# aliyun/heif-decoder-lib

Measured on AMD Instinct MI355X. Metric: megapixels/sec HEIC grid->RGB24, higher is better.
Workload: dtype u8

## Files before the change

heif-decoder-lib_amd/csrc/batch.cpp:

```cpp
#include <cstdio>
#include <algorithm>
#include <cmath>
#include <cstdlib>
#include <cstring>
#include <map>
#include <memory>
#include <tuple>
#include <vector>

#include "hm_device.h"
#include "hm_internal.h"
#include "hm_overlap_plan.h"

namespace {

struct DeviceBuffer {
  void* p = nullptr;
  size_t cap = 0;
  int ensure(size_t n)
  {
    if (n <= cap) return HM_OK;
    if (p) hm_pool_device_free(p);
    p = hm_pool_device_alloc(n);
    cap = p ? n : 0;
// ... 700 lines not shown
{
  if (!b) return hm_fail(HM_ERR_INVALID_ARG, "null batch");
  b->colour = false;
  b->tail_state = 0;
  b->col_y.clear(); b->col_cb.clear(); b->col_cr.clear(); b->col_out.clear();
  if (n_images == 0) return HM_OK;
  if (!d || n_images < 0 || !d_y || !d_cb || !d_cr || !d_out) return hm_fail(HM_ERR_INVALID_ARG, "null argument");
  if (b->items.empty() || b->items.size() % (size_t)n_images) return hm_fail(HM_ERR_INVALID_ARG, "%zu pictures do not divide into %d images", b->items.size(), n_images);
  const int pipe = hm_colour_pipeline(d);
  if (pipe < 0) return pipe;
  b->colour_desc = *d;
  b->col_y.assign(d_y, d_y + n_images); b->col_cb.assign(d_cb, d_cb + n_images); b->col_cr.assign(d_cr, d_cr + n_images);
  b->col_out.assign(d_out, d_out + n_images);
  b->colour_chunk = images_per_group;
  b->colour = true;
  return HM_OK;
}

int hm_batch_set_concurrency(hm_batch* b, int groups)
{
  if (!b || groups < 0 || groups > 8) return hm_fail(HM_ERR_INVALID_ARG, "bad argument");
  b->drain();
  b->groups = groups;
  return HM_OK;
}

int hm_batch_last_groups(const hm_batch* b, int* first_cut)
{
  if (!b) return -1;
  if (first_cut) *first_cut = b->last_cut;
  return b->last_groups;
}

int hm_batch_tail_kind(const hm_batch* b) { return b && b->tail_state == 2 ? b->tail_kind : -1; }

int hm_batch_tail_fused(const hm_batch* b) { return b && b->tail_state == 2 ? 1 : 0; }

int hm_batch_set_profiling(hm_batch* b, int slots)
{
  if (!b || slots < 0 || slots > 4096) return hm_fail(HM_ERR_INVALID_ARG, "bad argument");
  b->profiling = slots;
  b->exec_count = 0;
  return HM_OK;
}

static int batch_timings(hm_batch* b, int slot, float ms[5])
{
  if (!b || !ms) return hm_fail(HM_ERR_INVALID_ARG, "null argument");
  ms[0] = ms[1] = ms[2] = ms[3] = ms[4] = 0.f;
  if (!b->profiling || slot < 0 || slot >= b->profiling || slot >= b->exec_count || slot >= (int)b->timelines.size() || b->timelines[slot].used == 0)
    return hm_fail(HM_ERR_INVALID_ARG, "profiling not enabled or slot not recorded");
  const hm_batch::Timeline& t = b->timelines[slot];
  hipError_t e = hipEventSynchronize(t.ev[t.used - 1]);
  if (e != hipSuccess) return hm_check_hip(e, "hipEventSynchronize");
  if (t.spans) {
    std::vector<std::pair<float, float>> iv[5];
    for (size_t i = 1; i < t.used; i++) {
      if (t.kind[i] < 0) continue;
      float t0 = 0.f, t1 = 0.f;
      if ((e = hipEventElapsedTime(&t0, t.ev[0], t.ev[i - 1])) != hipSuccess || (e = hipEventElapsedTime(&t1, t.ev[0], t.ev[i])) != hipSuccess)
        return hm_check_hip(e, "hipEventElapsedTime");
      iv[t.kind[i]].emplace_back(t0, std::max(t0, t1));
    }
    for (int q = 0; q < 5; q++) {
      std::sort(iv[q].begin(), iv[q].end());
      float end = 0.f;
// ... 99 lines not shown
```

heif-decoder-lib_amd/csrc/chain.hip:

```cpp
#include "recon_common.h"

#include <stdlib.h>
#include <atomic>
#include <map>
#include <memory>
#include <mutex>
#include <new>
#include <utility>

#include "hm_internal.h"

namespace {

#ifdef HM_CHAIN_TIMING
#define HM_T_DECL unsigned long long t_prev = __builtin_amdgcn_s_memtime(); unsigned int t_acc[6] = {0, 0, 0, 0, 0, 0}, t_part[4] = {0, 0, 0, 0}; int t_in_svc = 0; (void)t_part; (void)t_in_svc
#if HM_CHAIN_TIMING == 2
#define HM_T_LAP(i) (void)t_prev
#define HM_T_COUNT(i) t_acc[i] += 64
#else
#define HM_T_LAP(i) do { if (HM_CHAIN_TIMING != 4) { const unsigned long long t_now = __builtin_amdgcn_s_memtime(); t_acc[i] += (unsigned int)(t_now - t_prev); t_prev = t_now; } } while (0)
#define HM_T_COUNT(i)
#endif
#if HM_CHAIN_TIMING == 4
#define HM_T_SVC_BEGIN() do { t_prev = __builtin_amdgcn_s_memtime(); t_in_svc = 1; } while (0)
// ... 584 lines not shown
          running = running && (uint32_t)my_off < my_kb;
          left = my_kb == 0 ? 0 : left;
          if (ballot(running) == 0) { __builtin_amdgcn_s_sleep(1); continue; }
        }
      }
    }
    const unsigned long long m_running = ballot(running);
    const int16_t* const my_res = rres + rslot * 16;
    const unsigned long long m_q4 = m_running & ballot((op.y & ((3u << OP_L2_SHIFT) | OP_INTERIOR)) == OP_INTERIOR);
    unsigned long long m_quad = m_q4, s_big = m_running & ~m_q4;
    int n_exec = 1, n_sub = 1;
    bool quad = running && (op.y & ((3u << OP_L2_SHIFT) | OP_INTERIOR)) == OP_INTERIOR;
    if (multi) {
      const uint32_t gq = (uint32_t)((m_q4 & 1) | ((m_q4 >> 15) & 2) | ((m_q4 >> 30) & 4) | ((m_q4 >> 45) & 8));
      const uint32_t gr = (uint32_t)((m_running & 1) | ((m_running >> 15) & 2) | ((m_running >> 30) & 4) | ((m_running >> 45) & 8));
      constexpr bool two = NCL == 1;
      constexpr int SUBX = CAN_LATE ? 2 : SUB;
      auto of_chain = [&](uint32_t m, int c) { return CAN_LATE ? ((m >> (2 * c)) & 3u) : (two ? (((m >> c) & 1u) | (((m >> (c + 2)) & 1u) << 1)) : (c ? 0u : m)); };
      uint32_t run[2], big[2];
#pragma unroll
      for (int c = 0; c < 2; c++) {
        const uint32_t q = of_chain(gq, c), r = of_chain(gr, c);
        run[c] = (uint32_t)__builtin_ctz(~q | (1u << SUBX));
        big[c] = (uint32_t)__builtin_ctz(~((r & ~q) >> run[c]));
      }
      const uint32_t my_run = g == 0 ? run[0] : run[1], my_big = g == 0 ? big[0] : big[1];
      quad = (uint32_t)my_off < my_run;
      m_quad = ballot(quad);
      s_big = ballot((uint32_t)my_off >= my_run && (uint32_t)my_off < my_run + my_big);
      n_exec = (int)(my_run + my_big);
      n_sub = (int)(run[0] > run[1] ? run[0] : run[1]);
    }
    (void)m_quad;
    const unsigned long long s_bres = s_big & ballot((op.y & (OP_CBF | (3u << OP_L2_SHIFT))) == (OP_CBF | (1u << OP_L2_SHIFT)));

    HM_T_LAP(1);
#if defined(HM_Q_PROBE) && (HM_Q_PROBE & 2048)
    if (s_bres && n_pics < 0) {
#else
    if (s_bres) {
#endif
      auto big_res = [&](int gg) -> uint32_t {
        uint32_t idx = (uint32_t)__builtin_amdgcn_readlane((int)op.z, gg * 16) + (uint32_t)lane;
        idx = idx < res_last ? idx : res_last;
        return (uint32_t)(int)resid[idx];
      };
      uint32_t sb_lo = (uint32_t)s_bres, sb_hi = (uint32_t)(s_bres >> 32);
      asm volatile("" : "+s"(sb_lo), "+s"(sb_hi));
      if (sb_lo & 0xFFFFu) bres0 = big_res(0);
      if (sb_lo >> 16) bres1 = big_res(1);
      if (sb_hi & 0xFFFFu) bres2 = big_res(2);
      if (sb_hi >> 16) bres3 = big_res(3);
    }

    HM_MARK("C_begin");
#if defined(HM_Q_PROBE) && (HM_Q_PROBE & 1)
    if (false) {
#else
    if (quad) {
#endif
      if (lane == (int)__builtin_ctzll(ballot(true))) HM_T_COUNT(3);
      const int res_q = (int)my_res[gl];
      const int mode = (int)(op.y & OP_MODE_MASK);
      const int P = Pk;
      Pix* const lp = gbase + (op.x & 0xFFFF);
      const Pix* const tbase = reinterpret_cast<const Pix*>(lds + ((op.y & OP_LINE) ? tl_off : gb_off));
      const Pix* const tc = tbase + (op.x >> 16);
// ... 45 lines not shown
        for (int t = 0; t < n_sub; t++) {
          if (my_off == t) execute();
          WAVE_SYNC();
        }
      }
      else execute();
    }
    WAVE_SYNC();

    HM_T_LAP(2);
    HM_MARK("D_begin");
#if defined(HM_Q_PROBE) && (HM_Q_PROBE & 2)
    for (unsigned long long todo = 0; todo;) {
#else
    for (unsigned long long todo = s_big; todo;) {
#endif
      const int bg = rfl((int)(__builtin_ctzll(todo) >> 4));
      todo &= ~(0xFFFFull << (bg * 16));
      HM_T_COUNT(4);
      const int src = bg * 16;
      const uint32_t ox = (uint32_t)__builtin_amdgcn_readlane((int)op.x, src), oy = (uint32_t)__builtin_amdgcn_readlane((int)op.y, src);
      const uint32_t oz = (uint32_t)__builtin_amdgcn_readlane((int)op.z, src), ow = (uint32_t)__builtin_amdgcn_readlane((int)op.w, src);
      const uint32_t s_gb = (uint32_t)__builtin_amdgcn_readlane((int)gb_off, src), s_tl = (uint32_t)__builtin_amdgcn_readlane((int)tl_off, src);
      const int mode = (int)(oy & OP_MODE_MASK), c = (int)((oy >> OP_C_SHIFT) & 3), log2 = 2 + (int)((oy >> OP_L2_SHIFT) & 3);
      const int path = (int)((oy >> OP_PATH_SHIFT) & 7);
#ifdef HM_D_SKIP
      if ((HM_D_SKIP >> (path != PATH_GEN ? path : 4 + log2)) & 1) continue;
#endif
#if defined(HM_Q_PROBE) && (HM_Q_PROBE & 512)
      const bool cbf = false;
#else
      const bool cbf = (oy & OP_CBF) != 0;
#endif
      const int P = c == 0 ? P0 : P1;
      Pix* const gb = reinterpret_cast<Pix*>(lds + s_gb);
      Pix* const lp = gb + (ox & 0xFFFF);
      const Pix* const tp = reinterpret_cast<const Pix*>(lds + ((oy & OP_LINE) ? s_tl : s_gb)) + (ox >> 16) + 1;
      Pix* const dst = lp + 1;
      const GLOBAL_AS int16_t* const gres = resid + oz;
      const int maxv = (1 << bd) - 1;

      HM_MARK("D_setup_end");
      auto block = [&](auto l2c, auto which) {
        constexpr int L2 = decltype(l2c)::value, WHICH = decltype(which)::value;
        int ln = lane;
        asm volatile("" : "+v"(ln));
        int res_s = 0, res_t[4] = {0, 0, 0, 0};
        const bool pairs = sizeof(Pix) == 1 && L2 >= 4 && WHICH != PATH_B4 && mode >= 2 && mode != 10 && mode != 26;
#ifdef HM_PAIRS_PRE
        uint32_t res_p[2] = {0, 0};
        if (cbf && pairs && L2 == 4) {
#pragma unroll
          for (int t = 0; t < 2; t++) res_p[t] = pairs8_residual<4>(mode >= 18, ln, t, gres);
        }
        else
#endif
        if (cbf && !pairs) {
          if (L2 == 2) {
            const int s_ri = __builtin_amdgcn_readlane((int)ri_me, src);
            const int s_chain = PAIRS ? bg & ((1 << NCL) - 1) : ((CAN_LATE && late) ? bg & 2 : bg);
            res_s = (int)(rres_all + s_chain * (RING * 16) + (s_ri & (RING - 1)) * 16)[ln & 15];
          }
          else if (L2 == 3) {
            uint32_t b = bg == 0 ? bres0 : (bg == 1 ? bres1 : (bg == 2 ? bres2 : bres3));
            asm volatile("" : "+v"(b));
            res_s = (int)b;
          }
          else if (L2 == 4) {
#pragma unroll
            for (int t = 0; t < 4; t++) res_t[t] = (int)gres[ln + 64 * t];
          }
        }
        auto emit = [&](int p, int x, int y, int v) {
          if (cbf) {
            int r;
            if (L2 <= 3) r = res_s;
            else if (L2 == 4) {
              const int t = rfl(p >> 6);
              r = t == 0 ? res_t[0] : (t == 1 ? res_t[1] : (t == 2 ? res_t[2] : res_t[3]));
            }
            else r = (int)gres[p];
            v = clip3i(0, maxv, v + r);
          }
          dst[mul24(y, P) + x] = (Pix)v;
        };
        Blk<Pix> B;
        B.mode = mode; B.c = c; B.bd = bd; B.log2 = L2; B.tskip = 0; B.qp = 0; B.n_coeff = 0; B.P = P;
        const bool smoothed = L2 != 2 && c == 0 && ((filter_mode_mask(L2) >> mode) & 1);
#if !defined(HM_Q_PROBE) || !(HM_Q_PROBE & 4)
        if (false) {}
        else if (WHICH == PATH_I16) {
          RefDirect<Pix> R;
          R.lp = lp; R.tp = tp; R.P = P;
          R.nL1 = (int)((oy >> OP_NL1_SHIFT) & 63); R.nT1 = (int)((oy >> OP_NT1_SHIFT) & 63);
          const int j = ln - 32;
          const int p = R(j), p_end = R(32);
          int pf = p;
          if (smoothed) {
            const int pm = dpp<0x138>(p);
            int pp = dpp<0x130>(p);
            pp = ln == 63 ? p_end : pp;
            pf = j == -32 ? p : (pm + 2 * p + pp + 2) >> 2;
          }
          int16_t* const bc = l_bA + 64;
          bc[j] = (int16_t)pf;
          if (ln == 0) bc[32] = (int16_t)p_end;
          WAVE_SYNC();
          if constexpr (sizeof(Pix) == 1 && L2 == 4) {
#ifdef HM_PAIRS_PRE
            if (pairs) predict_pairs8<4, true>(mode, bc, tab, ln, cbf, gres, reinterpret_cast<uint8_t*>(dst), P, res_p);
#else
            if (pairs) predict_pairs8<4, false>(mode, bc, tab, ln, cbf, gres, reinterpret_cast<uint8_t*>(dst), P);
#endif
            else predict_emit<Pix, L2>(B, RefArray{bc}, tab, ln, emit);
          }
          else predict_emit<Pix, L2>(B, RefArray{bc}, tab, ln, emit);
        }
        else if (WHICH == PATH_B4) {
          const uint32_t avail = ((ow & OPW_LEFT) ? 0xF0u : 0u) | (((ow >> OPW_BL_SHIFT) & 15) ? 0x0Fu : 0u) | ((ow & OPW_TL) ? 0x100u : 0u) |
                                 ((ow & OPW_TOP) ? 0x1E00u : 0u) | (((ow >> OPW_TR_SHIFT) & 15) ? 0x1E000u : 0u);
          const int b = ln < 16 ? ln : 16;
          const uint32_t lower = avail & ((1u << b) - 1u);
          const int first = avail ? (int)__builtin_ctz(avail) : 0;
          const int from = ((avail >> b) & 1u) ? b : (lower ? 31 - (int)__builtin_clz(lower) : first);
          const int j = from - 8;
          const Pix* const ql = lp + mul24_raw(-j - 1, P);
          const Pix* const qt = tp + (j - 1);
          int pv = *(j < 0 ? ql : qt);
          pv = avail ? pv : 1 << (bd - 1);
          int16_t* const bc = l_bA + 64;
          if (ln <= 16) bc[ln - 8] = (int16_t)pv;
          WAVE_SYNC();
          predict_emit<Pix, L2>(B, RefArray{bc}, tab, ln, emit);
        }
        else {
          constexpr uint32_t nT = 1u << L2;
          B.info = L2 | (c << HM_TU_CIDX_SHIFT) | ((ow & OPW_TL) ? HM_TU_AVAIL_TL : 0);
          B.aBL = (int)(((ow >> OPW_BL_SHIFT) & 15) << 2); B.aTR = (int)(((ow >> OPW_TR_SHIFT) & 15) << 2);
          B.avail = ((ow & OPW_LEFT) ? nT : 0u) | ((uint32_t)B.aBL << 8) | ((ow & OPW_TOP) ? nT << 16 : 0u) | ((uint32_t)B.aTR << 24);
          B.x0 = (int)((ow >> 6) & 0x3C); B.y0 = (int)((ow >> 10) & 0x3C);
          B.u = gb + (c == 2 ? cr_off : 0);
          B.top = reinterpret_cast<const Pix*>(lds + s_tl) + (c == 2 ? Wc + 4 : 0);
#if !defined(HM_Q_PROBE) || !(HM_Q_PROBE & 16)
          make_border<Pix, L2>(B, l_bA, strong, ln);
          WAVE_SYNC();
          if constexpr (sizeof(Pix) == 1 && L2 >= 4) {
            if (pairs) {
#ifdef HM_PAIRS_PRE
              if constexpr (L2 == 4) predict_pairs8<4, true>(mode, l_bA + 64, tab, ln, cbf, gres, reinterpret_cast<uint8_t*>(dst), P, res_p);
              else
#endif
              predict_pairs8<L2, false>(mode, l_bA + 64, tab, ln, cbf, gres, reinterpret_cast<uint8_t*>(dst), P);
            }
            else predict_emit<Pix, L2>(B, RefArray{l_bA + 64}, tab, ln, emit);
          }
          else predict_emit<Pix, L2>(B, RefArray{l_bA + 64}, tab, ln, emit);
#endif
        }
#endif
        if (L2 >= 4) __builtin_amdgcn_s_waitcnt(0x0F70);
        WAVE_SYNC();
        HM_MARK("D_pred_end");
      };
#if defined(HM_Q_PROBE) && (HM_Q_PROBE & 256)
      if (path == PATH_F8A) continue;
#endif
#if !defined(HM_Q_PROBE) || !(HM_Q_PROBE & 128)
      if (path == PATH_F8A) {
        int ln = lane;
        asm volatile("" : "+v"(ln));
        const int x = ln & 7, y = ln >> 3;
        const int nL1 = (int)((oy >> OP_NL1_SHIFT) & 63), nT1 = (int)((oy >> OP_NT1_SHIFT) & 63);
        const int angle = (int)(int8_t)(ow & 0xFF);
        const bool vert = mode >= 18;
        const int major = vert ? y : x, minor = vert ? x : y;
        const int t = mul24(major + 1, angle);
        const int f = t & 31, k = minor + (t >> 5);
        int r0, r1;
        if (angle > 0) {
          if (vert) { r0 = tp[imin_(k, nT1)]; r1 = tp[imin_(k + 1, nT1)]; }
          else { r0 = lp[mul24(imin_(k, nL1), P)]; r1 = lp[mul24(imin_(k + 1, nL1), P)]; }
        }
        else {
          const int inv = inv_angle_of(mode);
          const int k0 = k + 1, k1 = k + 2;
          const int q0 = -((mul24(k0, inv) + 128) >> 8), q1 = -((mul24(k1, inv) + 128) >> 8);
          const int j0 = k0 >= 0 ? k0 : q0, j1 = k1 >= 0 ? k1 : q1;
          auto at = [&](int j, bool main_side) -> int {
            const Pix* const qm = vert ? tp + imin_(j - 1, nT1) : lp + mul24(imin_(j - 1, nL1), P);
            const Pix* const qs = vert ? lp + mul24(imin_(-j - 1, nL1), P) : tp + imin_(-j - 1, nT1);
            return *(main_side ? qm : qs);
          };
          r0 = vert ? at(j0, j0 >= 0) : at(j0, j0 > 0);
          r1 = vert ? at(j1, j1 >= 0) : at(j1, j1 > 0);
        }
        int v = blend32(f, r0, r1);
        if (cbf) {
          uint32_t b = bg == 0 ? bres0 : (bg == 1 ? bres1 : (bg == 2 ? bres2 : bres3));
          asm volatile("" : "+v"(b));
          v = clip3i(0, maxv, v + (int)b);
        }
        dst[mul24(y, P) + x] = (Pix)v;
        WAVE_SYNC();
        continue;
      }
      else if (path == PATH_F8O) {
        int ln = lane;
        asm volatile("" : "+v"(ln));
        const int x = ln & 7, y = ln >> 3;
        const int nL1 = (int)((oy >> OP_NL1_SHIFT) & 63), nT1 = (int)((oy >> OP_NT1_SHIFT) & 63);
        const int t = tp[x], l = lp[mul24(y, P)];
        int v;
        if (mode == 0) v = planar_sample<3>(x, y, l, t, tp[imin_(8, nT1)], lp[mul24(imin_(8, nL1), P)]);
        else if (mode == 1) {
          int s2 = ln < 8 ? t : (ln < 16 ? (int)lp[mul24(ln - 8, P)] : 0);
          s2 += dpp<DPP_ROW_ROR(8)>(s2);
          s2 += dpp<DPP_ROW_ROR(4)>(s2);
          s2 += dpp<DPP_ROW_ROR(2)>(s2);
          s2 += dpp<DPP_ROW_ROR(1)>(s2);
          const int dc = (__builtin_amdgcn_readlane(s2, 0) + 8) >> 4;
          v = dc;
          if (c == 0) {
            const int dc3 = mad24_k<3>(dc, 2);
            v = y == 0 ? (t + dc3) >> 2 : v;
            v = x == 0 ? (l + dc3) >> 2 : v;
            v = (x | y) == 0 ? (l + 2 * dc + t + 2) >> 2 : v;
          }
        }
        else {
          const bool vert = mode == 26;
          v = vert ? t : l;
          if (c == 0) {
            const int corner = tp[-1];
            const int gq = vert ? (int)tp[0] + ((l - corner) >> 1) : (int)lp[0] + ((t - corner) >> 1);
            v = (vert ? x == 0 : y == 0) ? clip3i(0, maxv, gq) : v;
          }
        }
        if (cbf) {
          uint32_t b = bg == 0 ? bres0 : (bg == 1 ? bres1 : (bg == 2 ? bres2 : bres3));
          asm volatile("" : "+v"(b));
          v = clip3i(0, maxv, v + (int)b);
        }
        dst[mul24(y, P) + x] = (Pix)v;
        WAVE_SYNC();
        continue;
      }
      else if (path == PATH_S8) {
        int ln = lane;
        asm volatile("" : "+v"(ln));
        const int nL1 = (int)((oy >> OP_NL1_SHIFT) & 63), nT1 = (int)((oy >> OP_NT1_SHIFT) & 63);
        const int j = ln < 32 ? ln - 16 : 16;
        const Pix* const ql = lp + mul24_raw(imin_(-j - 1, nL1), P);
        const Pix* const qt = tp + imin_(j - 1, nT1);
        const int p = *(j < 0 ? ql : qt);
        const int pm = dpp<0x138>(p), pp = dpp<0x130>(p);
        const int pf = (j == -16 || j == 16) ? p : (pm + 2 * p + pp + 2) >> 2;
        int16_t* const bc = l_bA + 64;
        if (ln <= 32) bc[j] = (int16_t)pf;
        WAVE_SYNC();
        const int x = ln & 7, y = ln >> 3;
        int v;
        if (mode == 0) v = planar_sample<3>(x, y, bc[-1 - y], bc[1 + x], bc[9], bc[-9]);
        else v = bc[mode == 34 ? x + y + 2 : (mode == 2 ? -(x + y + 2) : x - y)];
        if (cbf) {
          uint32_t b = bg == 0 ? bres0 : (bg == 1 ? bres1 : (bg == 2 ? bres2 : bres3));
          asm volatile("" : "+v"(b));
          v = clip3i(0, maxv, v + (int)b);
        }
        dst[mul24(y, P) + x] = (Pix)v;
        WAVE_SYNC();
        continue;
      }
#endif
#if defined(HM_Q_PROBE) && (HM_Q_PROBE & 96)
      {
        const bool sm = log2 == 3 && c == 0 && ((filter_mode_mask(3) >> mode) & 1);
        const bool fast = log2 <= 3 && !sm && (oy & OP_INTERIOR);
        if (((HM_Q_PROBE & 32) && !fast) || ((HM_Q_PROBE & 64) && fast)) continue;
      }
#endif
      typedef std::integral_constant<int, PATH_GEN> gen_t;
      if (path == PATH_I16) block(std::integral_constant<int, 4>(), std::integral_constant<int, PATH_I16>());
      else if (path == PATH_B4) block(std::integral_constant<int, 2>(), std::integral_constant<int, PATH_B4>());
      else if (log2 == 3) block(std::integral_constant<int, 3>(), gen_t());
#if !defined(HM_Q_PROBE) || !(HM_Q_PROBE & 8)
      else if (log2 == 4) block(std::integral_constant<int, 4>(), gen_t());
      else block(std::integral_constant<int, 5>(), gen_t());
#endif
      WAVE_SYNC();
    }

#if defined(HM_PAD_S) || defined(HM_PAD_V)
    {
#ifdef HM_PAD_S
      int ps = lane0_dummy;
#pragma unroll
      for (int k = 0; k < HM_PAD_S; k++) asm volatile("s_add_u32 %0, %0, 1" : "+s"(ps));
      lane0_dummy = ps;
#endif
#ifdef HM_PAD_V
// ... 556 lines not shown
```

heif-decoder-lib_amd/csrc/hm_internal.h:

```cpp
#ifndef HM_INTERNAL_H
#define HM_INTERNAL_H

#include <hip/hip_runtime_api.h>

#include "heif_mi355x.h"

#ifdef __cplusplus
extern "C" {
#endif

int hm_check_hip(hipError_t e, const char* what);
int hm_fail(int status, const char* fmt, ...) __attribute__((format(printf, 2, 3)));
int hm_host_has_bmi2_lzcnt(void);
int hm_fail_detail(int status, int detail, const char* message);

int hm_launch_colour_int420(const hm_colour_desc* d, const int coef[4], const void* y, const void* cb,
                            const void* cr, void* out, hipStream_t s);
int hm_launch_colour_int420_batch(const hm_colour_desc* d, const int coef[4], int n, const void* const* y,
                                  const void* const* cb, const void* const* cr, void* const* out, hipStream_t s);
int hm_launch_colour_float(const hm_colour_desc* d, const float coef[4], int mode, const void* y,
                           const void* cb, const void* cr, void* out, hipStream_t s);
int hm_launch_to_hdr(const void* in, int in_stride, void* out, int out_stride, int w, int h, int out_bits, hipStream_t s);
int hm_launch_to_sdr(const void* in, int in_stride, void* out, int out_stride, int w, int h, int in_bits, hipStream_t s);
int hm_launch_set_alpha16(void* out, int out_stride, int w, int h, const void* alpha, int alpha_stride, int alpha_bits, int out_bits,
                          int big_endian, hipStream_t s);
int hm_launch_upsample_bilinear(int bit_depth, int v420, const void* in, int in_stride, void* out, int out_stride,
                                int w, int h, hipStream_t s);
int hm_launch_rotate_ccw(int bytes_per_sample, int angle, const void* in, int in_stride, int w, int h, void* out,
                         int out_stride, hipStream_t s);
int hm_launch_scale_nn(int bytes_per_sample, const void* in, int in_stride, int iw, int ih, void* out, int out_stride, int ow,
                       int oh, hipStream_t s);
int hm_launch_set_alpha(void* rgba, int out_stride, int w, int h, const void* alpha, int alpha_stride, hipStream_t s);
int hm_launch_mono_to_rgb(const void* y, int y_stride, void* out, int out_stride, int w, int h, int bpp, hipStream_t s);
int hm_launch_paste_bytes(const void* in, int in_stride, void* out, int out_stride, int copy_bytes, int rows, int rescale, int bit_depth,
                          int is_chroma, hipStream_t s);
int hm_launch_mirror(const void* in, int in_stride, int w, int h, int horizontal, void* out, int out_stride, hipStream_t s);

void* hm_pool_device_alloc(size_t bytes);
void hm_pool_device_free(void* p);
void* hm_pool_pinned_alloc(size_t bytes);
void hm_pool_pinned_free(void* p);
size_t hm_pool_device_cached(int device);
hipStream_t hm_pool_stream_get(void);
void hm_pool_stream_put(hipStream_t s, int device);

struct hm_dev_pic;
int hm_batch_add_trusted(hm_batch* b, const uint8_t* blob, size_t size, const hm_tile_dest* dest);
int hm_launch_recon(const struct hm_dev_pic* d_pics, int n_pics, int log2_ctb, int chroma_format, int bit_depth, int rare_syntax,
                    int max_ctb_w, int max_ctb_h, hipStream_t s);
int hm_launch_residual(const struct hm_dev_pic* d_pics, int n_pics, int max_ctb_h, hipStream_t s);
int hm_launch_chain(const struct hm_dev_pic* d_pics, int n_pics, int log2_ctb, int chroma_format, int bit_depth, int rare_syntax,
                    int max_ctb_w, int max_ctb_h, uint32_t* d_sync, size_t sync_bytes, uint32_t* d_err, hipStream_t s);
int hm_chain_plan(const struct hm_dev_pic* d_pics, int n_pics, int log2_ctb, int chroma_format, int bit_depth, int rare_syntax,
                  int max_ctb_w, int max_ctb_h, uint32_t* d_sync, size_t sync_bytes, uint32_t* d_err, int* per_picture, long* resident,
                  int* split_fraction);
int hm_batch_last_groups(const hm_batch* b, int* first_cut);
int hm_batch_tail_kind(const hm_batch* b);
int hm_tail_last_launch(void);
#include "hm_knobs.h"
size_t hm_chain_sync_bytes(int n_pics, int chroma_format, int max_ctb_h);
int hm_launch_deblock(const struct hm_dev_pic* d_pics, int n_pics, int max_w4, int max_h4, int chroma_format,
                      int bit_depth, int rare_syntax, hipStream_t s);
int hm_launch_sao_paste(const struct hm_dev_pic* d_pics, int n_pics, int max_w, int max_h, int bit_depth, int apply_sao,
                        int rare_syntax, hipStream_t s);
int hm_launch_tail420(const struct hm_dev_pic* d_pics, const void* d_dsts, int n_pics, int max_w, int max_h, int log2_ctb, int bpp, const int coef[4],
                      int stages, hipStream_t s);
int hm_colour_float_chain(const hm_colour_desc* d, float cf[4], int* mode);
int hm_launch_tailf(const struct hm_dev_pic* d_pics, const void* d_dsts, int n_pics, int max_w, int max_h, int log2_ctb, const hm_colour_desc* d, const float coef[4], int mode,
                    int stages, hipStream_t s);

HM_API long hm_parse_parallel_segments(int which);
HM_API int hm_debug_kernel_regs(int which, int a, int b, int c, int out[2]);
HM_API long hm_test_cabac_script(const uint8_t* data, size_t size, int qp, const int32_t* ops, int n_ops, uint32_t* out);

#ifdef __cplusplus
}
#endif
#endif
```

heif-decoder-lib_amd/csrc/recon_common.h:

```cpp
#ifndef HM_RECON_COMMON_H
#define HM_RECON_COMMON_H

#include <hip/hip_runtime.h>
#include <stdint.h>
#include <type_traits>

#include "hm_device.h"

namespace {

#define WAVE_SYNC()                                          \
  do {                                                       \
    __builtin_amdgcn_fence(__ATOMIC_ACQ_REL, "wavefront");  \
    __builtin_amdgcn_wave_barrier();                         \
  } while (0)

__device__ __forceinline__ int clip3i(int lo, int hi, int v) { return v < lo ? lo : (v > hi ? hi : v); }
__device__ __forceinline__ int iabs_(int v) { return v < 0 ? -v : v; }
__device__ __forceinline__ int imin_(int a, int b) { return a < b ? a : b; }
__device__ __forceinline__ int mul24(int a, int b) { return __mul24(a, b); }
__device__ __forceinline__ int mul24_raw(int a, int b)
{
  int d;
  asm("v_mul_i32_i24 %0, %1, %2" : "=v"(d) : "v"(a), "v"(b));
// ... 332 lines not shown
        const int t = mul24(major + 1, angle);
        const int k0 = minor + (t >> 5) + 1, iFact = t & 31;
        const int r0 = vert ? b.top(k0) : b.left(k0), r1 = vert ? b.top(k0 + 1) : b.left(k0 + 1);
        emit(p, x, y, blend32(iFact, r0, r1));
      });
    }
    else {
    const int inv = tab[35 + mode];
    lanes_loop<npx>(lane, [&](int p) {
      const int x = p & (nT - 1), y = p >> log2;
      const int major = vert ? y : x, minor = vert ? x : y;
      const int t = mul24(major + 1, angle);
      const int iIdx = t >> 5, iFact = t & 31;
      const int k0 = minor + iIdx + 1, k1 = k0 + 1;
      const int q0 = -((mul24(k0, inv) + 128) >> 8), q1 = -((mul24(k1, inv) + 128) >> 8);
      const int a0 = k0 >= 0 ? k0 : q0, a1 = k1 >= 0 ? k1 : q1;
      const int j0 = vert ? a0 : -a0, j1 = vert ? a1 : -a1;
      const int r0 = b(j0), r1 = b(j1);
      emit(p, x, y, blend32(iFact, r0, r1));
    });
    }
  }
}
template <int L2>
__device__ __forceinline__ uint32_t pairs8_residual(bool vert, int lane, int t, const GLOBAL_AS int16_t* gres)
{
  constexpr int nT = 1 << L2;
  const int q = lane + 64 * t;
  const int x = vert ? (q & (nT / 2 - 1)) << 1 : q & (nT - 1), y = vert ? q >> (L2 - 1) : (q >> L2) << 1;
  if (vert) return *reinterpret_cast<const GLOBAL_AS uint32_t*>(gres + (x + (y << L2)));
  return (uint32_t)(uint16_t)gres[x + (y << L2)] | ((uint32_t)(uint16_t)gres[x + ((y + 1) << L2)] << 16);
}
template <int L2, bool PRE = false>
__device__ __forceinline__ void predict_pairs8(int mode, const int16_t* bc, const int16_t* tab, int lane, bool cbf, const GLOBAL_AS int16_t* gres, uint8_t* dst, int P,
                                               const uint32_t* pre = nullptr)
{
  constexpr int nT = 1 << L2, TRIPS = nT * nT / 128;
  typedef short s16x2_t __attribute__((ext_vector_type(2)));
  typedef unsigned short u16x2_t __attribute__((ext_vector_type(2)));
  const int angle = __builtin_amdgcn_readfirstlane((int)tab[mode]);
  const int inv = __builtin_amdgcn_readfirstlane((int)tab[35 + mode]);
  const bool vert = mode >= 18;
  auto ref = [&](int k) -> uint32_t {
    const int a = k >= 0 ? k : -((mul24(k, inv) + 128) >> 8);
    return (uint32_t)(uint16_t)bc[vert ? a : -a];
  };
  auto ref_pos = [&](int k) -> uint32_t { return (uint32_t)(uint16_t)bc[vert ? k : -k]; };
  auto trip = [&](int t) {
    const int q = lane + 64 * t;
    const int major = vert ? q >> (L2 - 1) : q & (nT - 1);
    const int m0 = vert ? (q & (nT / 2 - 1)) << 1 : (q >> L2) << 1;
    const int tt = mul24(major + 1, angle);
    const int k0 = m0 + (tt >> 5) + 1;
    const uint32_t f = (uint32_t)(tt & 31);
    uint32_t r0, r1, r2;
    if (angle > 0) { r0 = ref_pos(k0); r1 = ref_pos(k0 + 1); r2 = ref_pos(k0 + 2); }
    else { r0 = ref(k0); r1 = ref(k0 + 1); r2 = ref(k0 + 2); }
    const uint32_t A = r0 | (r1 << 16), B = r1 | (r2 << 16);
    const uint32_t w1 = f | (f << 16), w0 = 0x00200020u - w1;
    u16x2_t v = __builtin_bit_cast(u16x2_t, A) * __builtin_bit_cast(u16x2_t, w0) + __builtin_bit_cast(u16x2_t, B) * __builtin_bit_cast(u16x2_t, w1) + (u16x2_t)(16);
    v = v >> (u16x2_t)(5);
    const int x = vert ? m0 : major, y = vert ? major : m0;
    if (cbf) {
      uint32_t rr;
      if constexpr (PRE) rr = pre[t];
      else rr = pairs8_residual<L2>(vert, lane, t, gres);
      s16x2_t s = __builtin_bit_cast(s16x2_t, v) + __builtin_bit_cast(s16x2_t, rr);
      s = __builtin_elementwise_min(__builtin_elementwise_max(s, (s16x2_t)(0)), (s16x2_t)(255));
      v = __builtin_bit_cast(u16x2_t, s);
    }
    const uint32_t vw = __builtin_bit_cast(uint32_t, v);
    uint8_t* const o = dst + mul24(y, P) + x;
    if (vert) *reinterpret_cast<uint16_t*>(o) = (uint16_t)((vw & 0xFFu) | ((vw >> 8) & 0xFF00u));
    else { o[0] = (uint8_t)vw; o[P] = (uint8_t)(vw >> 16); }
  };
  if constexpr (TRIPS <= 2) {
#pragma unroll
    for (int t = 0; t < TRIPS; t++) trip(t);
  }
  else {
#pragma unroll 2
    for (int t = 0; t < TRIPS; t++) trip(t);
  }
}

template <typename Pix, int L2, typename Ref, bool HALVES = false>
__device__ __forceinline__ void predict(const Blk<Pix>& B, const Ref& b, const int16_t* tab, int lane)
{
  Pix* const dst = B.u + mul24(B.y0, B.P) + UPAD + B.x0;
  const int pitch = B.P;
  predict_emit<Pix, L2, Ref, HALVES>(B, b, tab, lane, [&](int, int x, int y, int v) { dst[mul24(y, pitch) + x] = (Pix)v; });
}

struct ResidGeom {
  uint32_t luma_row, chroma_row, chroma_base, total;
  __device__ __forceinline__ uint32_t slab(int kind, int row) const { return kind ? chroma_base + (uint32_t)row * chroma_row : (uint32_t)row * luma_row; }
};
__device__ __forceinline__ ResidGeom resid_geom(int ctb_w, int ctb_h, int log2_ctb, int chroma_format)
{
  ResidGeom g;
  const uint32_t ctb = 1u << log2_ctb;
  g.luma_row = (uint32_t)ctb_w * ctb * ctb;
  g.chroma_row = chroma_format == 0 ? 0u : (uint32_t)ctb_w * 2u * (ctb >> 1) * (chroma_format == 1 ? ctb >> 1 : ctb);
  g.chroma_base = (uint32_t)ctb_h * g.luma_row;
  g.total = g.chroma_base + (uint32_t)ctb_h * g.chroma_row;
  return g;
}

constexpr uint32_t OP_MODE_MASK = 63u;
constexpr int OP_C_SHIFT = 6, OP_L2_SHIFT = 8;
constexpr uint32_t OP_CBF = 1u << 10, OP_INTERIOR = 1u << 11, OP_LINE = 1u << 13;
constexpr uint32_t OP_FAR = 1u << 26;
constexpr uint32_t OP_FAST8 = 1u << 12;
constexpr int OP_PATH_SHIFT = 27;
enum { PATH_GEN = 0,
       PATH_F8A = 1,
       PATH_F8O = 2,
       PATH_S8 = 3,
       PATH_I16 = 4,
       PATH_B4 = 5 };
constexpr uint32_t OP_SPECIAL = 1u << 31;
constexpr int OP_NL1_SHIFT = 14, OP_NT1_SHIFT = 20;
constexpr uint32_t OPW_LEFT = 1u << 16, OPW_TOP = 1u << 17, OPW_TL = 1u << 18;
constexpr int OPW_BL_SHIFT = 19, OPW_TR_SHIFT = 23;
typedef uint32_t mop_u32x4 __attribute__((ext_vector_type(4)));
__device__ __forceinline__ mop_u32x4 make_micro_op(uint32_t r0, unsigned a_left, unsigned a_top, unsigned a_tl, uint32_t aBL4, uint32_t aTR4, uint32_t qpy,
                                                   int Pk, int cr_off, int Wc, uint32_t roff)
{
  const int x4 = (int)(r0 & 15), y4 = (int)((r0 >> 4) & 15);
  const uint32_t info = (r0 >> 8) & 0xFF;
  const int l2 = (int)(info & HM_TU_LOG2_MASK), c = (int)((info >> HM_TU_CIDX_SHIFT) & 3);
  const uint32_t mode = (r0 >> 16) & OP_MODE_MASK;
  const bool cbf = (info & HM_TU_CBF) != 0;
  const int nT = 1 << l2;
  const bool left = a_left != 0, top = a_top != 0, tl = a_tl != 0;
  const int x0 = x4 << 2;
  const int lp = mul24(y4 << 2, Pk) + UPAD + x0 - 1 + (c == 2 ? cr_off : 0);
  const bool on_line = y4 == 0;
  const int tp = on_line ? x0 + (c == 2 ? Wc + 4 : 0) : lp - Pk;
  const uint32_t nL1 = (uint32_t)(nT - 1) + (aBL4 << 2), nT1 = (uint32_t)(nT - 1) + (aTR4 << 2);
  const bool interior = left && top && tl;
  const bool fast8 = l2 == 3 && interior && !(c == 0 && (mode == 0 || mode == 2 || mode == 18 || mode == 34));
  mop_u32x4 op;
  op.x = (uint32_t)lp | ((uint32_t)tp << 16);
  const bool special = mode <= 1 || (c == 0 && (mode == 10 || mode == 26));
// ... 190 lines not shown
```

heif-decoder-lib_amd/csrc/residual.hip:

```cpp
#include <cstdio>
#include <cstdlib>

#include "recon_common.h"
#include "hm_avail.h"

#include "hm_internal.h"
#include "residual_tables.h"

extern __device__ const hm_residual_tables hm_residual_tables_image;
__device__ const hm_residual_tables hm_residual_tables_image = hm_make_residual_tables();

namespace {

constexpr int R_WAVES = 4;
constexpr int R_TABLES_SMALL = 1024 + 256 + 128;
constexpr int R_STAGE = 256;
constexpr int R_WAVE = 2048 + 1024 + 4 * 16 * 4 + R_STAGE * 4;

template <int CTRL>
__device__ __forceinline__ int rdpp(int v) { return __builtin_amdgcn_update_dpp(0, v, CTRL, 0xF, 0xF, false); }
constexpr int R_ROW_ROR(int n) { return 0x120 | n; }
constexpr int R_QUAD_BCAST(int k) { return k | (k << 2) | (k << 4) | (k << 6); }

typedef short r_s16x2 __attribute__((ext_vector_type(2)));
// ... 247 lines not shown
      const int nT = 1 << l2;
      const int xin = x4 << 2, yc = k_row_y0 + (y4 << 2);
      const int ctb_pw = k_ctb_pw, rem_last = k_rem_last;
      const int room_x = (cnt_raw & HM_TU6_LAST_COLUMN) ? rem_last - (xin + nT) : ((info & HM_TU6_NEXT_TO_LAST) ? ctb_pw + rem_last - (xin + nT) : nT);
      const int room_y = k_plane_h - (yc + nT);
      const hm_avail av = hm_derive_avail(xin << lw, (y4 << 2) << lh, nT << lw, nT << lh, nT, room_x, room_y, dp.log2_ctb, (cnt_raw >> HM_TU6_NB_SHIFT) & 15u);
      mop = make_micro_op(r0, av.left, av.top, av.tl, (uint32_t)av.n_bl >> 2, (uint32_t)av.n_tr >> 2, 0u, m_Pk, m_cr_off, m_Wc, 0u);
      if (y4 == 0 && xin + nT + (int)(((uint32_t)av.n_tr >> 2) << 2) > ctb_pw) mop.y |= OP_FAR;
      asm volatile("" : "+v"(mop.x), "+v"(mop.y), "+v"(mop.w));
    }
    const bool cbf = valid && (info & HM_TU_CBF);
    const uint32_t rsz = (cbf && l2 >= 3) ? 16u << (2 * (l2 - 2)) : 0u;
    const uint32_t sc = wave_scan(cnt), sr = wave_scan(rsz);
    const uint32_t lo = lev_base + sc - cnt, ro = res_base + sr - rsz;
    mop.z = ro;
    const uint32_t n_lev = (uint32_t)__builtin_amdgcn_readlane((int)sc, 63);
    lev_base += n_lev;
    res_base += (uint32_t)__builtin_amdgcn_readlane((int)sr, 63);
    auto level = [&](uint32_t first, uint32_t i) -> uint32_t {
      const uint32_t rel = first - chunk_lev + i;
      uint32_t v;
      if (rel < (uint32_t)R_STAGE) v = lvl[rel];
      else {
        v = coeffs[first + i];
        asm volatile("" : "+v"(v));
      }
      return v;
    };
    __builtin_amdgcn_s_waitcnt(0x0F70);
#pragma unroll
    for (int k = 0; k < R_STAGE / 64; k++) lvl[lane + 64 * k] = staged[k];
    cur_x = ahead.x; cur_y = ahead.y;
    asm volatile("" : "+v"(cur_x), "+v"(cur_y));
    if (valid) mops[ri] = mop;
    if (kind == 0 && !(HM_R_SKIP & 32)) {
      if (cand_ok) {
        const uint32_t tf = cand_first - chunk;
        if (tf < 64u) __hip_atomic_fetch_add(slots + tf, 1, __ATOMIC_RELAXED, __HIP_MEMORY_SCOPE_WAVEFRONT);
      }
      WAVE_SYNC();
      int sm = slots[lane];
      WAVE_SYNC();
      slots[lane] = 0;
      sm = (int)wave_scan((uint32_t)sm);
      const int my_ctb = cur_ctb + sm;
      cur_ctb += __builtin_amdgcn_readlane(sm, 63);
      int lane_flags = __builtin_amdgcn_ds_bpermute((sm & 63) << 2, (int)ctb_flags);
      asm volatile("" : "+v"(lane_flags));
      if (sm >= 64) {
        lane_flags = (int)q0[HM_CTB_DWORDS * (size_t)my_ctb + 2];
        asm volatile("" : "+v"(lane_flags));
      }
      const int flags = valid ? (lane_flags & 0xFF) : 0;
      const int en = !(flags & HM_CTB_DEBLOCK_OFF);
      const int left_ok = ((x4 > 0) | ((flags & HM_CTB_DEBLOCK_LEFT) != 0)) & en;
      const int top_ok = ((y4 > 0) | ((flags & HM_CTB_DEBLOCK_TOP) != 0)) & en;
      const uint32_t qword = (((r0 >> 24) - (uint32_t)qp_bd_offset) & 0xFFu) << 8;
      const int l4 = dp.log2_ctb - 2;
      const int gx = (my_ctb << l4) + x4, gy = (row << l4) + y4;
      GLOBAL_AS uint16_t* const meta = gptr_w<uint16_t>(dp.meta);
      const int w4 = dp.w4, h4 = dp.h4;
      const uint32_t cell = (uint32_t)gx + __umul24((uint32_t)gy, (uint32_t)w4);
      const uint32_t top2 = (uint32_t)top_ok << 1;
      const bool inside = valid && gx < w4 && gy < h4;
      GLOBAL_AS uint32_t* const meta2 = reinterpret_cast<GLOBAL_AS uint32_t*>(meta);
      if (inside && l2 == 2) meta[cell] = (uint16_t)((uint32_t)left_ok | top2 | qword);
      if (inside && l2 == 3) {
        meta2[cell >> 1] = ((uint32_t)left_ok | top2 | qword) | ((top2 | qword) << 16);
        meta2[(cell + (uint32_t)w4) >> 1] = ((uint32_t)left_ok | qword) | (qword << 16);
      }
      const uint32_t pk = (uint32_t)left_ok | top2 | ((uint32_t)l2 << 2) | qword, gxy = (uint32_t)gx | ((uint32_t)gy << 16);
      for (unsigned long long mb = ballot(valid && l2 >= 4); mb; mb &= mb - 1) {
        const int b = (int)__builtin_ctzll(mb);
        const uint32_t s_pk = (uint32_t)__builtin_amdgcn_readlane((int)pk, b), s_gxy = (uint32_t)__builtin_amdgcn_readlane((int)gxy, b);
        const int s_l2 = (int)((s_pk >> 2) & 7), s_gx = (int)(s_gxy & 0xFFFFu), s_gy = (int)(s_gxy >> 16);
        const uint32_t s_q = s_pk & 0xFF00u;
        const int i = (lane & ((1 << (s_l2 - 3)) - 1)) << 1, j = lane >> (s_l2 - 3);
        if (lane < (1 << (2 * s_l2 - 5)) && s_gx + i < w4 && s_gy + j < h4) {
          const uint32_t t = j == 0 ? s_pk & 2u : 0u;
          meta2[((uint32_t)(s_gx + i) + __umul24((uint32_t)(s_gy + j), (uint32_t)w4)) >> 1] = ((i == 0 ? s_pk & 1u : 0u) | t | s_q) | ((t | s_q) << 16);
        }
      }
    }

    WAVE_SYNC();

    const uint32_t first_level = cbf ? level(lo, 0) : 0xFFFFu;
    const bool dc_only = cbf && cnt == 1 && (first_level & 0xFFFF) == 0 && !(info & HM_TU_TSKIP);
    auto dequant = [&](uint32_t raw, int qP, int l2b) -> int {
      const int q6 = (qP * 43) >> 8, qr = qP - 6 * q6;
      const int bdShift = bd + l2b - 9;
      const int32_t fact = (int32_t)tab[70 + qr] << q6;
      const int32_t prod = (int32_t)((uint32_t)mul24((int)(int16_t)(raw >> 16), fact) + (uint32_t)(1 << (bdShift - 1)));
      return clip3i(-32768, 32767, prod >> bdShift);
    };
    for (unsigned long long m4 = (HM_R_SKIP & 1) ? 0 : ballot(dc_only && l2 == 2); m4;) {
      int b[4];
#pragma unroll
      for (int k = 0; k < 4; k++) {
        b[k] = m4 ? (int)__builtin_ctzll(m4) : -1;
        m4 &= m4 - 1;
      }
      const int myb = g == 0 ? b[0] : (g == 1 ? b[1] : (g == 2 ? b[2] : b[3]));
      const bool act = myb >= 0;
      const int src = act ? myb : 0;
      const uint32_t br0 = (uint32_t)__shfl((int)r0, src), braw = (uint32_t)__shfl((int)first_level, src);
      const int c = dequant(braw, (int)(br0 >> 24), 2);
      const int m0y = kind ? 64 : (int)tab[76 + by_], m0x = kind ? 64 : (int)tab[76 + bx_];
      const int t1 = clip3i(-32768, 32767, (mul24(m0y, c) + 64) >> 7);
      int res = (mul24(m0x, t1) + rnd2) >> postShift;
      if (kind == 0) res = clip3i(-32768, 32767, res);
      if (act) res4[(size_t)(chunk + (uint32_t)myb) * 16 + (uint32_t)gl] = limit_res(res, maxv);
    }
    for (unsigned long long mdc = (HM_R_SKIP & 2) ? 0 : ballot(dc_only && l2 >= 3); mdc; mdc &= mdc - 1) {
      const int b = (int)__builtin_ctzll(mdc);
      const uint32_t s_r0 = (uint32_t)__builtin_amdgcn_readlane((int)r0, b), s_raw = (uint32_t)__builtin_amdgcn_readlane((int)first_level, b);
      const uint32_t s_ro = (uint32_t)__builtin_amdgcn_readlane((int)ro, b);
      const int s_l2 = (int)((s_r0 >> 8) & HM_TU_LOG2_MASK);
      const int c = dequant(s_raw, (int)(s_r0 >> 24), s_l2);
      const int t1 = clip3i(-32768, 32767, (64 * c + 64) >> 7);
      const int16_t k16 = limit_res((64 * t1 + rnd2) >> postShift, maxv);
      const uint32_t pair = (uint32_t)(uint16_t)k16 * 0x10001u;
      const int n_words = 1 << (2 * s_l2 - 1);
      GLOBAL_AS uint32_t* const out = reinterpret_cast<GLOBAL_AS uint32_t*>(resid + s_ro);
      for (int w = lane; w < n_words; w += 64) out[w] = pair;
    }

    for (unsigned long long m4 = (HM_R_SKIP & 4) ? 0 : ballot(cbf && l2 == 2 && !dc_only); m4;) {
      int b[4];
#pragma unroll
      for (int k = 0; k < 4; k++) {
        b[k] = m4 ? (int)__builtin_ctzll(m4) : -1;
        m4 &= m4 - 1;
      }
      const int myb = g == 0 ? b[0] : (g == 1 ? b[1] : (g == 2 ? b[2] : b[3]));
      const bool act = myb >= 0;
      const int src = act ? myb : 0;
      const uint32_t br0 = (uint32_t)__shfl((int)r0, src), bcnt = (uint32_t)__shfl((int)cnt, src);
      const uint32_t blo = (uint32_t)__shfl((int)lo, src);
      const bool has = act && (uint32_t)gl < bcnt;
      uint32_t raw = 0;
      if (has) raw = level(blo, (uint32_t)gl);
      const int qP = (int)(br0 >> 24);
      const int q6 = (qP * 43) >> 8, qr = qP - 6 * q6;
      const int bdShift = bd - 7;
      const int32_t fact = (int32_t)tab[70 + qr] << q6;
      const int pos = (int)(raw & 15);
      if (has) {
        const int value = (int)(int16_t)(raw >> 16);
        const int32_t prod = (int32_t)((uint32_t)mul24(value, fact) + (uint32_t)(1 << (bdShift - 1)));
        slots[g * 16 + pos] = clip3i(-32768, 32767, prod >> bdShift);
      }
      WAVE_SYNC();
      const int cq = slots[g * 16 + gl];
      WAVE_SYNC();
      if (has) slots[g * 16 + pos] = 0;
      int res;
      if ((br0 >> 8) & HM_TU_TSKIP) {
// ... 98 lines not shown
```

Measured before the change: 159,000.

## Encode DC-only large residual blocks as constant in op instead of filling buffer

For DC-only transform units of size 8x8 and larger, the residual stage now computes the single constant residual value and stores it in the op descriptor with a new OP_CONST flag, instead of writing the whole block of identical residuals to global memory. The reconstruction kernel checks the flag and adds the constant directly in every prediction path, including the paired 8-bit path, skipping global residual loads for those blocks. This removes global writes and reads but adds branches in the hot reconstruction code. It also moves the DC computation before the mop store, and adds a debug helper that reads mops back to the host.

```diff
diff --git a/heif-decoder-lib_amd/csrc/batch.cpp b/heif-decoder-lib_amd/csrc/batch.cpp
--- a/heif-decoder-lib_amd/csrc/batch.cpp
+++ b/heif-decoder-lib_amd/csrc/batch.cpp
@@ -756,6 +756,22 @@
   return b->last_groups;
 }
 
+long hm_batch_read_mops(hm_batch* b, int item, uint32_t* out, long capacity)
+{
+  if (!b || (!out && capacity > 0) || item < 0 || item >= (int)b->items.size() || !b->uploaded) return -1;
+  b->drain();
+  for (const Class& c : b->classes)
+    for (size_t k = 0; k < c.items.size(); k++) {
+      if (c.items[k] != item) continue;
+      const hm_dev_pic& dp = b->h_desc[c.desc_offset + k];
+      const long n = dp.mops ? (long)b->items[item].hdr.n_tus : 0;
+      const long take = n < capacity ? n : capacity;
+      if (take > 0 && hipMemcpy(out, dp.mops, (size_t)take * 16, hipMemcpyDeviceToHost) != hipSuccess) return -1;
+      return n;
+    }
+  return -1;
+}
+
 int hm_batch_tail_kind(const hm_batch* b) { return b && b->tail_state == 2 ? b->tail_kind : -1; }
 
 int hm_batch_tail_fused(const hm_batch* b) { return b && b->tail_state == 2 ? 1 : 0; }
diff --git a/heif-decoder-lib_amd/csrc/chain.hip b/heif-decoder-lib_amd/csrc/chain.hip
--- a/heif-decoder-lib_amd/csrc/chain.hip
+++ b/heif-decoder-lib_amd/csrc/chain.hip
@@ -640,7 +640,7 @@
       n_sub = (int)(run[0] > run[1] ? run[0] : run[1]);
     }
     (void)m_quad;
-    const unsigned long long s_bres = s_big & ballot((op.y & (OP_CBF | (3u << OP_L2_SHIFT))) == (OP_CBF | (1u << OP_L2_SHIFT)));
+    const unsigned long long s_bres = s_big & ballot((op.y & (OP_CBF | OP_CONST | (3u << OP_L2_SHIFT))) == (OP_CBF | (1u << OP_L2_SHIFT)));
 
     HM_T_LAP(1);
 #if defined(HM_Q_PROBE) && (HM_Q_PROBE & 2048)
@@ -752,6 +752,8 @@
 #else
       const bool cbf = (oy & OP_CBF) != 0;
 #endif
+      auto konst = [&]() { return (oy & OP_CONST) != 0; };
+      auto kres = [&]() { return (int)(int16_t)oz; };
       const int P = c == 0 ? P0 : P1;
       Pix* const gb = reinterpret_cast<Pix*>(lds + s_gb);
       Pix* const lp = gb + (ox & 0xFFFF);
@@ -767,16 +769,24 @@
         asm volatile("" : "+v"(ln));
         int res_s = 0, res_t[4] = {0, 0, 0, 0};
         const bool pairs = sizeof(Pix) == 1 && L2 >= 4 && WHICH != PATH_B4 && mode >= 2 && mode != 10 && mode != 26;
+        const uint32_t kpair = (oz & 0xFFFFu) | (oz << 16);
 #ifdef HM_PAIRS_PRE
         uint32_t res_p[2] = {0, 0};
-        if (cbf && pairs && L2 == 4) {
+        if (cbf && !konst() && pairs && L2 == 4) {
 #pragma unroll
           for (int t = 0; t < 2; t++) res_p[t] = pairs8_residual<4>(mode >= 18, ln, t, gres);
         }
         else
 #endif
         if (cbf && !pairs) {
-          if (L2 == 2) {
+          if (L2 >= 3 && konst()) {
+            if (L2 == 3) res_s = kres();
+            else if (L2 == 4) {
+#pragma unroll
+              for (int t = 0; t < 4; t++) res_t[t] = kres();
+            }
+          }
+          else if (L2 == 2) {
             const int s_ri = __builtin_amdgcn_readlane((int)ri_me, src);
             const int s_chain = PAIRS ? bg & ((1 << NCL) - 1) : ((CAN_LATE && late) ? bg & 2 : bg);
             res_s = (int)(rres_all + s_chain * (RING * 16) + (s_ri & (RING - 1)) * 16)[ln & 15];
@@ -799,6 +809,7 @@
               const int t = rfl(p >> 6);
               r = t == 0 ? res_t[0] : (t == 1 ? res_t[1] : (t == 2 ? res_t[2] : res_t[3]));
             }
+            else if (konst()) r = kres();
             else r = (int)gres[p];
             v = clip3i(0, maxv, v + r);
           }
@@ -828,9 +839,9 @@
           WAVE_SYNC();
           if constexpr (sizeof(Pix) == 1 && L2 == 4) {
 #ifdef HM_PAIRS_PRE
-            if (pairs) predict_pairs8<4, true>(mode, bc, tab, ln, cbf, gres, reinterpret_cast<uint8_t*>(dst), P, res_p);
+            if (pairs) predict_pairs8<4, true>(mode, bc, tab, ln, cbf, konst(), kpair, gres, reinterpret_cast<uint8_t*>(dst), P, res_p);
 #else
-            if (pairs) predict_pairs8<4, false>(mode, bc, tab, ln, cbf, gres, reinterpret_cast<uint8_t*>(dst), P);
+            if (pairs) predict_pairs8<4, false>(mode, bc, tab, ln, cbf, konst(), kpair, gres, reinterpret_cast<uint8_t*>(dst), P);
 #endif
             else predict_emit<Pix, L2>(B, RefArray{bc}, tab, ln, emit);
           }
@@ -867,10 +878,10 @@
           if constexpr (sizeof(Pix) == 1 && L2 >= 4) {
             if (pairs) {
 #ifdef HM_PAIRS_PRE
-              if constexpr (L2 == 4) predict_pairs8<4, true>(mode, l_bA + 64, tab, ln, cbf, gres, reinterpret_cast<uint8_t*>(dst), P, res_p);
+              if constexpr (L2 == 4) predict_pairs8<4, true>(mode, l_bA + 64, tab, ln, cbf, konst(), kpair, gres, reinterpret_cast<uint8_t*>(dst), P, res_p);
               else
 #endif
-              predict_pairs8<L2, false>(mode, l_bA + 64, tab, ln, cbf, gres, reinterpret_cast<uint8_t*>(dst), P);
+              predict_pairs8<L2, false>(mode, l_bA + 64, tab, ln, cbf, konst(), kpair, gres, reinterpret_cast<uint8_t*>(dst), P);
             }
             else predict_emit<Pix, L2>(B, RefArray{l_bA + 64}, tab, ln, emit);
           }
@@ -916,9 +927,12 @@
         }
         int v = blend32(f, r0, r1);
         if (cbf) {
-          uint32_t b = bg == 0 ? bres0 : (bg == 1 ? bres1 : (bg == 2 ? bres2 : bres3));
-          asm volatile("" : "+v"(b));
-          v = clip3i(0, maxv, v + (int)b);
+          if (konst()) v = clip3i(0, maxv, v + kres());
+          else {
+            uint32_t b = bg == 0 ? bres0 : (bg == 1 ? bres1 : (bg == 2 ? bres2 : bres3));
+            asm volatile("" : "+v"(b));
+            v = clip3i(0, maxv, v + (int)b);
+          }
         }
         dst[mul24(y, P) + x] = (Pix)v;
         WAVE_SYNC();
@@ -957,9 +971,12 @@
           }
         }
         if (cbf) {
-          uint32_t b = bg == 0 ? bres0 : (bg == 1 ? bres1 : (bg == 2 ? bres2 : bres3));
-          asm volatile("" : "+v"(b));
-          v = clip3i(0, maxv, v + (int)b);
+          if (konst()) v = clip3i(0, maxv, v + kres());
+          else {
+            uint32_t b = bg == 0 ? bres0 : (bg == 1 ? bres1 : (bg == 2 ? bres2 : bres3));
+            asm volatile("" : "+v"(b));
+            v = clip3i(0, maxv, v + (int)b);
+          }
         }
         dst[mul24(y, P) + x] = (Pix)v;
         WAVE_SYNC();
@@ -983,9 +1000,12 @@
         if (mode == 0) v = planar_sample<3>(x, y, bc[-1 - y], bc[1 + x], bc[9], bc[-9]);
         else v = bc[mode == 34 ? x + y + 2 : (mode == 2 ? -(x + y + 2) : x - y)];
         if (cbf) {
-          uint32_t b = bg == 0 ? bres0 : (bg == 1 ? bres1 : (bg == 2 ? bres2 : bres3));
-          asm volatile("" : "+v"(b));
-          v = clip3i(0, maxv, v + (int)b);
+          if (konst()) v = clip3i(0, maxv, v + kres());
+          else {
+            uint32_t b = bg == 0 ? bres0 : (bg == 1 ? bres1 : (bg == 2 ? bres2 : bres3));
+            asm volatile("" : "+v"(b));
+            v = clip3i(0, maxv, v + (int)b);
+          }
         }
         dst[mul24(y, P) + x] = (Pix)v;
         WAVE_SYNC();
diff --git a/heif-decoder-lib_amd/csrc/hm_internal.h b/heif-decoder-lib_amd/csrc/hm_internal.h
--- a/heif-decoder-lib_amd/csrc/hm_internal.h
+++ b/heif-decoder-lib_amd/csrc/hm_internal.h
@@ -55,6 +55,7 @@
                   int max_ctb_w, int max_ctb_h, uint32_t* d_sync, size_t sync_bytes, uint32_t* d_err, int* per_picture, long* resident,
                   int* split_fraction);
 int hm_batch_last_groups(const hm_batch* b, int* first_cut);
+long hm_batch_read_mops(hm_batch* b, int item, uint32_t* out, long capacity);
 int hm_batch_tail_kind(const hm_batch* b);
 int hm_tail_last_launch(void);
 #include "hm_knobs.h"
diff --git a/heif-decoder-lib_amd/csrc/recon_common.h b/heif-decoder-lib_amd/csrc/recon_common.h
--- a/heif-decoder-lib_amd/csrc/recon_common.h
+++ b/heif-decoder-lib_amd/csrc/recon_common.h
@@ -388,8 +388,8 @@
   return (uint32_t)(uint16_t)gres[x + (y << L2)] | ((uint32_t)(uint16_t)gres[x + ((y + 1) << L2)] << 16);
 }
 template <int L2, bool PRE = false>
-__device__ __forceinline__ void predict_pairs8(int mode, const int16_t* bc, const int16_t* tab, int lane, bool cbf, const GLOBAL_AS int16_t* gres, uint8_t* dst, int P,
-                                               const uint32_t* pre = nullptr)
+__device__ __forceinline__ void predict_pairs8(int mode, const int16_t* bc, const int16_t* tab, int lane, bool cbf, bool konst, uint32_t kpair,
+                                               const GLOBAL_AS int16_t* gres, uint8_t* dst, int P, const uint32_t* pre = nullptr)
 {
   constexpr int nT = 1 << L2, TRIPS = nT * nT / 128;
   typedef short s16x2_t __attribute__((ext_vector_type(2)));
@@ -418,10 +418,14 @@
     v = v >> (u16x2_t)(5);
     const int x = vert ? m0 : major, y = vert ? major : m0;
     if (cbf) {
-      uint32_t rr;
-      if constexpr (PRE) rr = pre[t];
-      else rr = pairs8_residual<L2>(vert, lane, t, gres);
-      s16x2_t s = __builtin_bit_cast(s16x2_t, v) + __builtin_bit_cast(s16x2_t, rr);
+      s16x2_t s;
+      if (konst) s = __builtin_bit_cast(s16x2_t, v) + __builtin_bit_cast(s16x2_t, kpair);
+      else {
+        uint32_t rr;
+        if constexpr (PRE) rr = pre[t];
+        else rr = pairs8_residual<L2>(vert, lane, t, gres);
+        s = __builtin_bit_cast(s16x2_t, v) + __builtin_bit_cast(s16x2_t, rr);
+      }
       s = __builtin_elementwise_min(__builtin_elementwise_max(s, (s16x2_t)(0)), (s16x2_t)(255));
       v = __builtin_bit_cast(u16x2_t, s);
     }
@@ -467,6 +471,7 @@
 constexpr int OP_C_SHIFT = 6, OP_L2_SHIFT = 8;
 constexpr uint32_t OP_CBF = 1u << 10, OP_INTERIOR = 1u << 11, OP_LINE = 1u << 13;
 constexpr uint32_t OP_FAR = 1u << 26;
+constexpr uint32_t OP_CONST = 1u << 30;
 constexpr uint32_t OP_FAST8 = 1u << 12;
 constexpr int OP_PATH_SHIFT = 27;
 enum { PATH_GEN = 0,
diff --git a/heif-decoder-lib_amd/csrc/residual.hip b/heif-decoder-lib_amd/csrc/residual.hip
--- a/heif-decoder-lib_amd/csrc/residual.hip
+++ b/heif-decoder-lib_amd/csrc/residual.hip
@@ -303,6 +303,23 @@
     for (int k = 0; k < R_STAGE / 64; k++) lvl[lane + 64 * k] = staged[k];
     cur_x = ahead.x; cur_y = ahead.y;
     asm volatile("" : "+v"(cur_x), "+v"(cur_y));
+    WAVE_SYNC();
+    const uint32_t first_level = cbf ? level(lo, 0) : 0xFFFFu;
+    const bool dc_only = cbf && cnt == 1 && (first_level & 0xFFFF) == 0 && !(info & HM_TU_TSKIP);
+    auto dequant = [&](uint32_t raw, int qP, int l2b) -> int {
+      const int q6 = (qP * 43) >> 8, qr = qP - 6 * q6;
+      const int bdShift = bd + l2b - 9;
+      const int32_t fact = (int32_t)tab[70 + qr] << q6;
+      const int32_t prod = (int32_t)((uint32_t)mul24((int)(int16_t)(raw >> 16), fact) + (uint32_t)(1 << (bdShift - 1)));
+      return clip3i(-32768, 32767, prod >> bdShift);
+    };
+    if (!(HM_R_SKIP & 2) && dc_only && l2 >= 3) {
+      const int c = dequant(first_level, (int)(r0 >> 24), l2);
+      const int t1 = clip3i(-32768, 32767, (64 * c + 64) >> 7);
+      const int16_t k16 = limit_res((64 * t1 + rnd2) >> postShift, maxv);
+      mop.y |= OP_CONST;
+      mop.z = (uint32_t)(uint16_t)k16;
+    }
     if (valid) mops[ri] = mop;
     if (kind == 0 && !(HM_R_SKIP & 32)) {
       if (cand_ok) {
@@ -356,15 +373,6 @@
 
     WAVE_SYNC();
 
-    const uint32_t first_level = cbf ? level(lo, 0) : 0xFFFFu;
-    const bool dc_only = cbf && cnt == 1 && (first_level & 0xFFFF) == 0 && !(info & HM_TU_TSKIP);
-    auto dequant = [&](uint32_t raw, int qP, int l2b) -> int {
-      const int q6 = (qP * 43) >> 8, qr = qP - 6 * q6;
-      const int bdShift = bd + l2b - 9;
-      const int32_t fact = (int32_t)tab[70 + qr] << q6;
-      const int32_t prod = (int32_t)((uint32_t)mul24((int)(int16_t)(raw >> 16), fact) + (uint32_t)(1 << (bdShift - 1)));
-      return clip3i(-32768, 32767, prod >> bdShift);
-    };
     for (unsigned long long m4 = (HM_R_SKIP & 1) ? 0 : ballot(dc_only && l2 == 2); m4;) {
       int b[4];
 #pragma unroll
@@ -382,19 +390,6 @@
       int res = (mul24(m0x, t1) + rnd2) >> postShift;
       if (kind == 0) res = clip3i(-32768, 32767, res);
       if (act) res4[(size_t)(chunk + (uint32_t)myb) * 16 + (uint32_t)gl] = limit_res(res, maxv);
-    }
-    for (unsigned long long mdc = (HM_R_SKIP & 2) ? 0 : ballot(dc_only && l2 >= 3); mdc; mdc &= mdc - 1) {
-      const int b = (int)__builtin_ctzll(mdc);
-      const uint32_t s_r0 = (uint32_t)__builtin_amdgcn_readlane((int)r0, b), s_raw = (uint32_t)__builtin_amdgcn_readlane((int)first_level, b);
-      const uint32_t s_ro = (uint32_t)__builtin_amdgcn_readlane((int)ro, b);
-      const int s_l2 = (int)((s_r0 >> 8) & HM_TU_LOG2_MASK);
-      const int c = dequant(s_raw, (int)(s_r0 >> 24), s_l2);
-      const int t1 = clip3i(-32768, 32767, (64 * c + 64) >> 7);
-      const int16_t k16 = limit_res((64 * t1 + rnd2) >> postShift, maxv);
-      const uint32_t pair = (uint32_t)(uint16_t)k16 * 0x10001u;
-      const int n_words = 1 << (2 * s_l2 - 1);
-      GLOBAL_AS uint32_t* const out = reinterpret_cast<GLOBAL_AS uint32_t*>(resid + s_ro);
-      for (int w = lane; w < n_words; w += 64) out[w] = pair;
     }
 
     for (unsigned long long m4 = (HM_R_SKIP & 4) ? 0 : ballot(cbf && l2 == 2 && !dc_only); m4;) {
```

After: 160,300 (median of 6 runs). No clear change (+0.9%).
